# roitberg-group/lammps-ani

Hardware: AMD Instinct MI355X
Metric: MD ns/day for ANI-2x water box (0.5 fs steps; whole timestep loop: integrate + re-neighbour + ghost exchange + pair_style ani hot path) (higher is better)
Workload: dtype f32

## Files before the change

lammps-ani_amd/csrc/ani_handle.h:

```cpp
#pragma once
#include "../../include/ani_hip.h"
#include "../../include/ani_comm.h"

#include <hip/hip_runtime.h>
#ifndef ANI_NO_ROCTX
#include <rocprofiler-sdk-roctx/roctx.h>
#else
static inline void roctxRangePushA(const char*) {}
static inline void roctxRangePop() {}
static inline void roctxMarkA(const char*) {}
#endif

#include <algorithm>
#include <atomic>
#include <chrono>
#include <cmath>
#include <cstdio>
#include <cstdlib>
#include <cstring>
#include <string>
#include <vector>

#include "ani_kernels.h"
#include "ani_model.h"
// ... 43 lines not shown
  std::vector<double*> W64, b64, WT64;
  double *W0c64 = nullptr, *WT0c64 = nullptr, *w_out64 = nullptr, *b_out64 = nullptr;
  struct Planes {
    std::vector<unsigned short*> W, WT;
    unsigned short *W0c = nullptr, *WT0c = nullptr;
  } sp[2];
  std::vector<float> wscale;
  struct Fused {
    unsigned char* stream = nullptr;
    float* consts = nullptr;
    long long ppm = 0;
    int cpm = 0;
  } fu[4];
  int fused_shape = -1;
};
inline MlpArith planes_arith(int i) { return i == 0 ? MLP_BF16X3 : MLP_F16X2; }

struct Options {
  int prune = 1;
  int mlp_pipeline = 0;
  int aev_fused = 1;
  int aev_sym_radial = 1;
  int aev_tickets_min = 40000;
  int aev_stream_tables = 1;
  int mlp_fused_sched = 1;
  int mlp_fused_halves = 1;
  int mlp_fused = 1;
  int mlp_fused_gen = 1;
  int mlp_fused_rows = 0;
  int mlp_chain = 1;
  int profiling = 0;
  int dev_overwrite = 0;
  int mlp_arith = MLP_BF16X3;
  int rdf_lanes = 16, rdf_lds = 1;
  int nbr_onepass = 1, nbr_sorted_rows = 1, nbr_half_cells = 0;
  int reuse_upload = 0;
  int out_force_accumulate = 0;
};

struct FusedState {
  int mask[4] = {-2, -2, -2, -2};
  DevBuf<int> counter;
  DevBuf<int> sched;
  int sched_key[4] = {-1, -1, -1, -1};
  int sched_nitems = 0;
  DevBuf<float> gaev_parts;
// ... 117 lines not shown
  int split_phase = 0;
  hipStream_t side = nullptr;
  hipEvent_t ev_mlp = nullptr, ev_side = nullptr;
  struct { const double* d_x; int eflag_atom, vflag; double *d_f, *d_ev, *d_eatom; } split{};
  int nlocal = 0, ntotal = 0, nrows = 0;
  long long npairs = 0;
  int count[kMaxSpecies] = {0}, row_start[kMaxSpecies] = {0};

  ani_comm* comm = nullptr;
  int sticky_flags = 0;
  int max_numneigh = 0;
  DevBuf<int> species, ilist, numneigh, jlist, jraw, nbr_off, row_of_centre, centre_of_row, bucket_info, err_flag;
  DevBuf<int> row_of_atom;
  DevBuf<unsigned> sym_acc;
  int jraw_stride = 0;
  int jlist_row_stride = 0;
  const int64_t* stage_owner = nullptr;
  const double* stage_shift = nullptr;
  int stage_nghost = -1;
  bool origin_from_box = false;
  GhostFold fold;
  int fold_nghost = -1;
  DevBuf<int> fold_head, fold_next, fold_bad;
  bool warned_asymmetric = false;
  bool list_is_ours = false;
  bool list_symmetric = true;
  DevBuf<int> row_ctr;
  DevBuf<float4> xyzs, cl_xyz;
  DevBuf<int4> row_info, cl_hdr;
  DevBuf<int> cl_j;
  int cl_stride = 0;
  DevBuf<double> x64, f64, ev, eatom, virial_acc;
  DevBuf<double> origin;
  bool need_origin = true;
  DevBuf<double> rep_tables, erep;
  DevBuf<float> aev, gaev, act, e_rows, fbuf;
  DevBuf<double> aev64, gaev64, act64, e_rows64, fbuf64;
  std::vector<std::vector<double*>> Hbuf64;
  std::vector<std::vector<float*>> Hbuf, Gbuf;
  bool arena_valid = false;
};

#define HIP_TRY(h, expr)                                                                              \
  do {                                                                                                \
    hipError_t _e = (expr);                                                                           \
    if (_e != hipSuccess) {                                                                           \
// ... 83 lines not shown
```

lammps-ani_amd/csrc/ani_hip.cpp:

```cpp
#include "ani_handle.h"

namespace ani {
static thread_local hipError_t g_launch_error = hipSuccess;
void note_launch_error(hipError_t e) { if (e != hipSuccess && g_launch_error == hipSuccess) g_launch_error = e; }
hipError_t take_launch_error() { const hipError_t e = g_launch_error; g_launch_error = hipSuccess; return e; }
}

namespace ani_host __attribute__((visibility("hidden"))) {
thread_local std::string g_create_error;
constexpr int kCopyOutBlocks = 32;

int run_step64(ani_handle* h, const double* d_x, int eflag_atom, int vflag, double* d_f, int f_accumulate, double* d_ev,
               double* d_eatom, hipStream_t st) {
  const HostModel& m = h->model;
  const int L = m.L, M = m.M;
  HIP_TRY(h, h->fbuf64.reserve((size_t)std::max(h->ntotal, 1) * 3));
  HIP_TRY(h, h->virial_acc.reserve(9 * kVirialSlots));
  HIP_TRY(h, h->err_flag.reserve(1, true));
  HIP_TRY(h, hipMemsetAsync(h->fbuf64.p, 0, sizeof(double) * 3 * (size_t)h->ntotal, st));
  HIP_TRY(h, hipMemsetAsync(h->virial_acc.p, 0, sizeof(double) * 9, st));
  HIP_TRY(h, hipMemsetAsync(h->e_rows64.p, 0, sizeof(double) * (size_t)M * std::max(h->nrows, 1), st));
  if (h->armed.av_acc) HIP_TRY(h, hipMemsetAsync(h->armed.av_acc, 0, sizeof(double) * 9 * (size_t)h->ntotal, st));
  Aev64Params p{};
  const AevParams& r = h->ap_run;
// ... 208 lines not shown
  StreamTab tab_view;
  const bool rep_done = launch_aev_backward(h->ap_run, a, h->max_numneigh, st, rt.on ? &rt : nullptr, avir, step_stream_tab(h, tab_view)) && rt.on;
  if (m.has_rep && !rep_done) {
    RepArgs ra{};
    ra.row_info = h->row_info.p; ra.nrows = h->nrows; ra.jlist = h->jlist.p; ra.species = h->species.p;
    ra.pos = c.d_x; ra.fbuf = h->fbuf.p; ra.virial = c.vflag ? h->virial_acc.p : nullptr; ra.erep = h->erep.p;
    ra.tables = h->rep_tables.p; ra.S = m.S; ra.nslots = kVirialSlots; ra.vslots = kVirialSlots; ra.cutoff = m.rep_cut;
    launch_repulsion(ra, false, st, avir);
  }
  return ANI_OK;
}

void step_finish(ani_handle* h, const StepCtx& c, int atom0, int atom1, bool energy, hipStream_t st) {
  const HostModel& m = h->model;
  FinishArgs fa{};
  fa.e_rows = h->e_rows.p; fa.M = m.M; fa.nrows = h->nrows; fa.nrows_ld = h->nrows;
  fa.centre_of_row = h->centre_of_row.p; fa.ilist = h->ilist.p; fa.species = h->species.p;
  for (int s = 0; s < m.S; s++) fa.sae[s] = m.sae[s];
  fa.fbuf = h->fbuf.p; fa.atom0 = atom0; fa.atom1 = atom1; fa.energy = energy ? 1 : 0;
  fa.virial_acc = c.vflag ? h->virial_acc.p : nullptr;
  fa.f_out = c.d_f; fa.f_accumulate = c.f_accumulate; fa.ev_out = c.d_ev;
  fa.eatom_out = c.eflag_atom ? c.d_eatom : nullptr;
  fa.err_flag = h->err_flag.p;
  if (h->fold_nghost >= 0 && c.fold) {
    fa.fold_head = h->fold_head.p; fa.fold_next = h->fold_next.p; fa.fold_nlocal = h->nlocal;
    fa.atom1 = std::min(fa.atom1, h->nlocal);
  }
  launch_finish(fa, st);
  if (energy && m.has_rep) launch_repulsion_energy(h->erep.p, kVirialSlots, c.d_ev, st);
}

int run_step(ani_handle* h, const double* d_x, int eflag_atom, int vflag, double* d_f, int f_accumulate, double* d_ev,
             double* d_eatom, hipStream_t st, bool fold = false) {
  if (!h->use_single) return run_step64(h, d_x, eflag_atom, vflag, d_f, f_accumulate, d_ev, d_eatom, st);
  StepCtx c;
  c.fold = fold;
  c.d_x = d_x; c.eflag_atom = eflag_atom; c.vflag = vflag; c.f_accumulate = f_accumulate; c.d_f = d_f; c.d_ev = d_ev; c.d_eatom = d_eatom;
  TraceRange tr_step("ani: step");
  int rc = step_prologue(h, c, true, st);
  if (rc) return rc;
  step_pack(h, c, 0, h->ntotal, true, st);
  if (h->armed.av_acc) HIP_TRY(h, hipMemsetAsync(h->armed.av_acc, 0, sizeof(float) * 9 * (size_t)h->ntotal, st));
  const AevArgs a = step_aev_args(h, c, 0);
  rc = step_compact_forward(h, a, st);
  if (rc) return rc;
  {
    TraceRange tr("ani: MLP forward + backward");
    rc = compute_mlp(h, st);
// ... 170 lines not shown
  for (auto& n : h->nets) {
    for (float* p : n.W) if (p) (void)hipFree(p);
    for (float* p : n.b) if (p) (void)hipFree(p);
    for (float* p : n.WT) if (p) (void)hipFree(p);
    if (n.W0c) (void)hipFree(n.W0c);
    if (n.WT0c) (void)hipFree(n.WT0c);
    if (n.w_out) (void)hipFree(n.w_out);
    if (n.b_out) (void)hipFree(n.b_out);
    for (auto& sp : n.sp) {
      for (unsigned short* p : sp.W) if (p) (void)hipFree(p);
      for (unsigned short* p : sp.WT) if (p) (void)hipFree(p);
      if (sp.W0c) (void)hipFree(sp.W0c);
      if (sp.WT0c) (void)hipFree(sp.WT0c);
    }
    for (double* p : n.W64) if (p) (void)hipFree(p);
    for (double* p : n.b64) if (p) (void)hipFree(p);
    for (double* p : n.WT64) if (p) (void)hipFree(p);
    if (n.W0c64) (void)hipFree(n.W0c64);
    if (n.WT0c64) (void)hipFree(n.WT0c64);
    if (n.w_out64) (void)hipFree(n.w_out64);
    if (n.b_out64) (void)hipFree(n.b_out64);
  }
  h->species.release(); h->ilist.release(); h->numneigh.release(); h->jlist.release(); h->jraw.release(); h->nbr_off.release();
  h->fold_head.release(); h->fold_next.release(); h->fold_bad.release(); h->nb.ovf.release(); h->nb.xq.release(); h->row_of_centre.release(); h->centre_of_row.release(); h->bucket_info.release(); h->err_flag.release(); h->row_ctr.release(); h->row_of_atom.release();
  h->xyzs.release(); h->cl_xyz.release(); h->cl_hdr.release(); h->cl_j.release(); h->row_info.release(); h->row_flag.release(); h->row_list.release(); h->row_count.release(); h->x64.release(); h->f64.release(); h->ev.release(); h->eatom.release(); h->origin.release();
  h->rep_tables.release(); h->erep.release();
  h->nb.cell_id.release(); h->nb.cell_count.release(); h->nb.cell_start.release(); h->nb.cursor.release(); h->nb.order.release(); h->nb.xs.release();
  h->armed.avir.release(); h->armed.avir64.release(); h->armed.avout.release();
  h->armed.gaev_parts64.release(); h->armed.dv_fbuf.release(); h->armed.dv_fbuf64.release(); h->armed.dv_tmp.release(); h->armed.dv_stage.release();
  h->armed.dv_part.release(); h->armed.dv_ticket.release();
  h->mol.bond_cut2.release(); h->mol.ints.release(); h->mol.words.release(); h->mol.owner.release(); h->mol.summary.release(); h->mol.out.release();
  h->rdf.ints.release(); h->rdf.words.release();
  h->virial_acc.release(); h->aev.release(); h->gaev.release(); h->act.release(); h->aev64.release(); h->gaev64.release(); h->act64.release(); h->e_rows64.release(); h->fbuf64.release(); h->e_rows.release(); h->fbuf.release();
  for (int fi = 0; fi < 4; fi++) free_fused(h, fi);
  h->fused.counter.release(); h->fused.gaev_parts.release(); h->fused.sched.release();
  h->stab.desc_b.release(); h->stab.desc_f.release(); h->stab.words_b.release(); h->stab.words_f.release();
  free_chain_plan(h->chain_plan);
  for (auto& e : h->timing.evt_pool) if (e) (void)hipEventDestroy(e);
  if (h->stream) (void)hipStreamDestroy(h->stream);
  delete h;
}

const char* ani_last_error(const ani_handle* h) { return h ? h->err.c_str() : g_create_error.c_str(); }
int ani_num_models(const ani_handle* h) { return h ? h->model.M_file : 0; }
int ani_use_num_models(const ani_handle* h) { return h ? h->model.M : 0; }
int ani_num_species(const ani_handle* h) { return h ? h->model.S : 0; }
int ani_aev_length(const ani_handle* h) { return h ? h->model.aev_len : 0; }
// ... 263 lines not shown
```

lammps-ani_amd/csrc/ani_hip_list.cpp:

```cpp
#include "ani_handle.h"

namespace ani_host __attribute__((visibility("hidden"))) {
constexpr int kRebuildRowsOverflow = -1000;
int rebuild(ani_handle* h, hipStream_t st) {
  const HostModel& m = h->model;
  roctxMarkA("neighbor list rebuilt");
  TraceRange tr("ani: list epoch set-up (offsets, species buckets, segment sort)");
  h->need_origin = !h->origin_from_box;
  h->fold_nghost = -1;
  h->classes_valid = false;
  h->split_phase = 0;
  const int nlocal = h->nlocal;
  const int nrows_cap = round_up(nlocal, kRowTile) + m.S * kRowTile;
  HIP_TRY(h, h->nbr_off.reserve((size_t)nlocal + 1));
  HIP_TRY(h, h->row_of_centre.reserve(prepare_scratch_ints(nlocal)));
  HIP_TRY(h, h->centre_of_row.reserve(nrows_cap));
  HIP_TRY(h, h->row_info.reserve(nrows_cap));
  HIP_TRY(h, h->bucket_info.reserve(kBucketInfoInts));
  HIP_TRY(h, h->err_flag.reserve(1, true));
  if (!h->host.pinned_ints) HIP_TRY(h, hipHostMalloc((void**)&h->host.pinned_ints, sizeof(int) * 32, hipHostMallocDefault));
  h->host.pinned_ints[0] = h->host.pinned_ints[1] = h->host.pinned_ints[2] = 0;
  HIP_TRY(h, hipMemcpyAsync(&h->host.pinned_ints[0], h->err_flag.p, sizeof(int), hipMemcpyDeviceToHost, st));
  HIP_TRY(h, hipMemsetAsync(h->err_flag.p, 0, sizeof(int), st));
  HIP_TRY(h, h->row_of_atom.reserve((size_t)std::max(h->ntotal, 1)));
  PrepOut o{h->nbr_off.p, h->row_of_centre.p, h->centre_of_row.p, h->row_info.p, h->bucket_info.p, h->row_of_atom.p};
  launch_prepare(h->species.p, h->ilist.p, h->numneigh.p, nlocal, h->ntotal, m.S, nrows_cap, o, st, h->jlist_row_stride);
  if (h->jlist_row_stride) HIP_TRY(h, hipMemcpyAsync(&h->host.pinned_ints[1], h->nb.ovf.p, sizeof(int), hipMemcpyDeviceToHost, st));
  const bool fold_staged = h->stage_nghost >= 0 && h->stage_owner && h->use_single && h->stage_nghost == h->ntotal - nlocal;
  if (fold_staged) {
    HIP_TRY(h, h->fold_head.reserve((size_t)std::max(nlocal, 1)));
    HIP_TRY(h, h->fold_next.reserve((size_t)std::max(h->stage_nghost, 1)));
    HIP_TRY(h, h->fold_bad.reserve(1));
    launch_ghost_chain(reinterpret_cast<const long long*>(h->stage_owner), h->stage_nghost, nlocal, h->fold_head.p, h->fold_next.p, h->fold_bad.p, st);
    HIP_TRY(h, hipMemcpyAsync(&h->host.pinned_ints[2], h->fold_bad.p, sizeof(int), hipMemcpyDeviceToHost, st));
  }
  int info[kBucketInfoInts];
  HIP_TRY(h, hipMemcpyAsync(info, h->bucket_info.p, sizeof(info), hipMemcpyDeviceToHost, st));
  HIP_TRY(h, hipStreamSynchronize(st));
  h->sticky_flags |= h->host.pinned_ints[0];
  HIP_TRY(h, take_launch_error());
  if (h->jlist_row_stride && h->host.pinned_ints[1]) return kRebuildRowsOverflow;
  if (h->jlist_row_stride) h->npairs = info[2 * kMaxSpecies + 4];
  if (fold_staged) {
    if (h->host.pinned_ints[2]) { h->stage_nghost = -1; h->err = "ani_stage_ghost_fold: an owner index lies outside [0, nlocal)"; return ANI_ERR_ARG; }
    h->fold.owner = reinterpret_cast<const long long*>(h->stage_owner); h->fold.shift = h->stage_shift; h->fold.nlocal = nlocal;
    h->fold_nghost = h->stage_nghost;
  }
  h->stage_nghost = -1;
  if (info[2 * kMaxSpecies + 1]) { h->err = "an atom has a species outside the model's species list (or ilist holds an index outside [0, ntotal))"; return ANI_ERR_ARG; }
  for (int s = 0; s < m.S; s++) { h->count[s] = info[s]; h->row_start[s] = info[kMaxSpecies + s]; }
  h->nrows = info[2 * kMaxSpecies];
  h->max_numneigh = info[2 * kMaxSpecies + 2];
  {
    const int rcs = specialize(h, info[2 * kMaxSpecies + 3]);
    if (rcs) return rcs;
    const int rct = build_stream_tables(h, st);
// ... 218 lines not shown
  h->host.species32.resize(ntotal);
  for (int i = 0; i < ntotal; i++) h->host.species32[i] = (int)species[i];
  HIP_TRY(h, h->species.reserve(ntotal));
  HIP_TRY(h, h->x64.reserve((size_t)ntotal * 3));
  HIP_TRY(h, hipMemcpyAsync(h->species.p, h->host.species32.data(), sizeof(int) * (size_t)ntotal, hipMemcpyHostToDevice, st));
  HIP_TRY(h, hipMemcpyAsync(h->x64.p, coordinates, sizeof(double) * 3 * (size_t)ntotal, hipMemcpyHostToDevice, st));
  const int rcb = build_list(h, ntotal, nlocal, h->species.p, h->x64.p, cutneigh, lo, hi, out_npairs, st);
  h->host.x64_from = (rcb == ANI_OK && h->opt.reuse_upload) ? coordinates : nullptr;
  return rcb;
}

int ani_set_ghost_fold(ani_handle* h, const int64_t* d_owner, const double* d_shift, int nghost, void* stream) {
  if (!h) return ANI_ERR_ARG;
  if (!d_owner || nghost < 0) { h->fold_nghost = -1; return ANI_OK; }
  if (!h->use_single) { h->err = "ani_set_ghost_fold: the fp64 kernels do not fold ghosts (use the exchange kernels)"; return ANI_ERR_ARG; }
  if (!h->have_list || nghost != h->ntotal - h->nlocal) { h->err = "ani_set_ghost_fold: no list installed, or nghost differs from the list's"; return ANI_ERR_ARG; }
  if (!d_shift && nghost > 0) { h->err = "ani_set_ghost_fold: null shift"; return ANI_ERR_ARG; }
  HIP_TRY(h, hipSetDevice(h->device));
  hipStream_t st = (hipStream_t)stream;
  HIP_TRY(h, h->fold_head.reserve((size_t)std::max(h->nlocal, 1)));
  HIP_TRY(h, h->fold_next.reserve((size_t)std::max(nghost, 1)));
  HIP_TRY(h, h->fold_bad.reserve(1));
  static_assert(sizeof(long long) == sizeof(int64_t), "owner indices are 64-bit");
  launch_ghost_chain(reinterpret_cast<const long long*>(d_owner), nghost, h->nlocal, h->fold_head.p, h->fold_next.p, h->fold_bad.p, st);
  int bad = 0;
  HIP_TRY(h, hipMemcpyAsync(&bad, h->fold_bad.p, sizeof(int), hipMemcpyDeviceToHost, st));
  HIP_TRY(h, hipStreamSynchronize(st));
  HIP_TRY(h, take_launch_error());
  if (bad) { h->fold_nghost = -1; h->err = "ani_set_ghost_fold: an owner index lies outside [0, nlocal)"; return ANI_ERR_ARG; }
  h->fold.owner = reinterpret_cast<const long long*>(d_owner); h->fold.shift = d_shift; h->fold.nlocal = h->nlocal;
  h->fold_nghost = nghost;
  return ANI_OK;
}

int ani_stage_ghost_fold(ani_handle* h, const int64_t* d_owner, const double* d_shift, int nghost) {
  if (!h) return ANI_ERR_ARG;
  h->stage_owner = nullptr; h->stage_shift = nullptr; h->stage_nghost = -1;
  if (!d_owner || nghost < 0) return ANI_OK;
  if (!h->use_single) { h->err = "ani_stage_ghost_fold: the fp64 kernels do not fold ghosts (use the exchange kernels)"; return ANI_ERR_ARG; }
  if (!d_shift && nghost > 0) { h->err = "ani_stage_ghost_fold: null shift"; return ANI_ERR_ARG; }
  h->stage_owner = d_owner; h->stage_shift = d_shift; h->stage_nghost = nghost;
  return ANI_OK;
}
}
```

lammps-ani_amd/csrc/ani_hip_options.cpp:

```cpp
#include "ani_handle.h"

extern "C" {
void ani_trace_push(const char* name) { if (name) roctxRangePushA(name); }
void ani_trace_pop(void) { roctxRangePop(); }
void ani_trace_mark(const char* name) { if (name) roctxMarkA(name); }

const char* ani_last_mlp_kernel(const ani_handle* h) { return h ? h->last_mlp_kernel : ""; }

int ani_debug_get(ani_handle* h, ani_debug_view* out) {
  if (!h || !out) return ANI_ERR_ARG;
  memset(out, 0, sizeof(*out));
  out->nlocal = h->nlocal; out->ntotal = h->ntotal; out->nrows = h->nrows; out->npairs = h->npairs;
  out->d_aev = h->aev.p; out->d_gaev = h->gaev.p; out->d_row_of_centre = h->row_of_centre.p;
  out->aev_stride = h->ap_run.aev_stride; out->aev_active_length = h->ap_run.aev_len;
  if (h->err_flag.p) {
    int flag = 0;
    if (hipSetDevice(h->device) == hipSuccess && hipDeviceSynchronize() == hipSuccess &&
        hipMemcpy(&flag, h->err_flag.p, sizeof(int), hipMemcpyDeviceToHost) == hipSuccess)
      h->sticky_flags |= flag;
  }
  out->error_flags = h->sticky_flags;
  for (int s = 0; s < kMaxSpecies && s < 16; s++) out->species_count[s] = h->count[s];
  return ANI_OK;
}
// ... 39 lines not shown
  for (int c = 0; c < h->ap_run.aev_len && c < (int)h->colmap.size(); c++) out[c] = h->colmap[c];
  return ANI_OK;
}

enum OptKind { kFlag, kRange, kSet };
enum OptInvalidates { kNothing, kSchedule, kList, kUpload };
struct OptRow { const char* name; int Options::*field; OptKind kind; int v[3]; const char* refusal; OptInvalidates invalidates; };
constexpr int kAny = 0x7fffffff;
static const OptRow kOptionRows[] = {
    {"prune_absent_species", &Options::prune, kFlag, {}, nullptr, kList},
    {"rdf_lanes", &Options::rdf_lanes, kSet, {16, 64, 64}, "ani_set_option: rdf_lanes is 16 or 64", kNothing},
    {"rdf_lds", &Options::rdf_lds, kFlag, {}, nullptr, kNothing},
    {"mlp_chain", &Options::mlp_chain, kRange, {-kAny - 1, kAny}, nullptr, kNothing},
    {"nbr_onepass", &Options::nbr_onepass, kFlag, {}, nullptr, kNothing},
    {"out_force_accumulate", &Options::out_force_accumulate, kFlag, {}, nullptr, kNothing},
    {"nbr_sorted_rows", &Options::nbr_sorted_rows, kFlag, {}, nullptr, kNothing},
    {"nbr_half_cells", &Options::nbr_half_cells, kFlag, {}, nullptr, kNothing},
    {"reuse_build_list_upload", &Options::reuse_upload, kFlag, {}, nullptr, kUpload},
    {"mlp_fused", &Options::mlp_fused, kRange, {0, 3}, "mlp_fused must be 0, 1, 2 or 3", kNothing},
    {"aev_symmetric_radial", &Options::aev_sym_radial, kFlag, {}, nullptr, kNothing},
    {"aev_tickets_min", &Options::aev_tickets_min, kRange, {0, kAny}, "aev_tickets_min must be >= 0", kNothing},
    {"aev_fused", &Options::aev_fused, kFlag, {}, nullptr, kNothing},
    {"aev_stream_tables", &Options::aev_stream_tables, kFlag, {}, nullptr, kNothing},
    {"mlp_fused_gen", &Options::mlp_fused_gen, kRange, {0, 1}, "mlp_fused_gen must be 0 or 1", kSchedule},
    {"mlp_fused_rows", &Options::mlp_fused_rows, kSet, {0, 64, 128}, "mlp_fused_rows must be 0, 64 or 128", kSchedule},
    {"mlp_fused_halves", &Options::mlp_fused_halves, kRange, {0, 2}, "mlp_fused_halves must be 0, 1 or 2", kSchedule},
    {"mlp_fused_schedule", &Options::mlp_fused_sched, kFlag, {}, nullptr, kSchedule},
    {"mlp_pipeline", &Options::mlp_pipeline, kRange, {0, 2}, "mlp_pipeline must be 0, 1 or 2", kNothing},
    {"mlp_arith", &Options::mlp_arith, kRange, {0, 2}, "mlp_arith must be 0 (fp32-input MFMA), 1 (bf16 x 3, exact) or 2 (fp16 x 2)", kNothing},
    {"mlp_split_bf16", &Options::mlp_arith, kFlag, {}, nullptr, kNothing},
    {"device_overwrite_forces", &Options::dev_overwrite, kFlag, {}, nullptr, kNothing},
    {"profiling", &Options::profiling, kFlag, {}, nullptr, kNothing},
    {"full_radial_capacity", nullptr, kFlag, {}, nullptr, kNothing},
};
static_assert(MLP_FP32 == 0 && MLP_BF16X3 == 1, "mlp_split_bf16 is a flag onto mlp_arith");

int ani_set_option(ani_handle* h, const char* name, int value) {
  if (!h || !name) return ANI_ERR_ARG;
  for (const OptRow& r : kOptionRows) {
    if (strcmp(name, r.name) != 0) continue;
    const bool ok = r.kind == kFlag || (r.kind == kRange ? value >= r.v[0] && value <= r.v[1] : value == r.v[0] || value == r.v[1] || value == r.v[2]);
    if (!ok) { h->err = r.refusal; return ANI_ERR_ARG; }
    const int stored = r.kind == kFlag ? value != 0 : value;
    if (r.field) h->opt.*r.field = stored;
    else h->ap.full_cap = h->ap_run.full_cap = stored;
    if (r.invalidates == kSchedule) h->fused.sched_key[0] = -1;
// ... 92 lines not shown
```

lammps-ani_amd/csrc/ani_kernels.h:

```cpp
#pragma once
#include <hip/hip_runtime.h>

#include <cstdint>
#include <vector>

#include "ani_fused_host.h"
#include "ani_model.h"

namespace ani {

constexpr int kRowTile = 128;
constexpr int kMaxRad = 256;
constexpr int kMaxAng = 96;
constexpr int kBucketInfoInts = 2 * kMaxSpecies + 5;
constexpr int kVirialSlots = 1024;

enum Epilogue { EPI_PLAIN = 0, EPI_CELU = 1, EPI_LAST = 2, EPI_BWD = 3 };

void note_launch_error(hipError_t e);
hipError_t take_launch_error();
int device_num_cus();
hipError_t raise_dynamic_lds(const void* kernel, int bytes);

struct GemmArgs {
// ... 70 lines not shown
void launch_build_stream(const float* src, int ld, int rows_valid, int k_valid, int NT, int KS, int chunk, int P, float scale,
                         unsigned short* dst, hipStream_t st);
hipError_t launch_mlp_fused(const FusedArgs& G, MlpArith arith, hipStream_t st);
hipError_t launch_mlp_fused16(const FusedArgs& G, MlpArith arith, int waves, hipStream_t st);
int fused16_b1_chunks(int nt0);
int fused16_b1_chunk_tiles(int nt0, int ci);
void launch_build_stream16(const float* src, int ld, int rows_valid, int k_valid, int NT, int KS, int order, int nt_off, int identity,
                           int P, float scale, unsigned short* dst, hipStream_t st);
void launch_sum_parts(const float* parts, long long part_stride, int M, float* dst, long long n, hipStream_t st);
int aev_read_stamps(unsigned long long* out32, int reset);
int fused_read_stamps(unsigned long long* out16, int reset);

void launch_split_planes(const float* src, int batch, long long s_src, int N, int K, int ld, MlpArith arith, float scale,
                         unsigned short* dst, hipStream_t st);
inline size_t split_elems(int N, int K, MlpArith arith) { return (size_t)N * ((K + 15) / 16) * 16 * mlp_planes(arith); }

struct SpeciesMap { int m[kMaxSpecies]; };
void launch_origin(const double* d_x, int ntotal, double* d_origin, hipStream_t st);
struct GhostFold {
  const long long* owner = nullptr;
  const double* shift = nullptr;
  int nlocal = 0;
};
void launch_ghost_chain(const long long* d_owner, int nghost, int nlocal, int* d_head, int* d_next, int* d_bad, hipStream_t st);
void launch_pack(const double* d_x, const int* d_species, int i0, int i1, const SpeciesMap& cmap, float4* xyzs, float* fbuf,
                 double* virial_acc, double* ev_zero, const double* d_origin, hipStream_t st, const GhostFold* gf = nullptr);
void launch_row_classes(const int4* row_info, const int* jlist, int nrows, int nlocal, int* flag, int* list, int* count, hipStream_t st);

void launch_step_tail(const double* d_ev, const int* d_flag, double* host_out, double stamp, hipStream_t st);
void launch_copy_out(const double* d_f, double* host, long long n, int nchunks, unsigned long long* d_ctr, unsigned* host_flags,
                     unsigned epoch, int nblocks, hipStream_t st);

struct PrepOut {
  int* nbr_off;
  int* row_of_centre;
  int* centre_of_row;
  int4* row_info;
  int* bucket_info;
  int* row_of_atom;
};
size_t prepare_scratch_ints(int nlocal);
void launch_prepare(const int* d_species, const int* d_ilist, const int* d_numneigh, int nlocal, int ntotal, int S, int nrows_cap,
                    const PrepOut& o, hipStream_t st, int row_stride = 0);
void launch_list_symmetry(const int* d_ilist, const int* d_nbr_off, const int* d_numneigh, const int* d_jraw, const int* d_row_of_atom,
                          int nlocal, int ntotal, unsigned* d_acc, int* d_out, hipStream_t st);

constexpr int kTicketGroups = 64;
constexpr int kTicketMaxGroups = 256;
static_assert(kTicketGroups <= kTicketMaxGroups, "kTicketGroups");
constexpr int kTicketStride = 64;
struct AevArgs {
  const float4* xyzs;
  const int* ilist;
  const int* numneigh;
  const int* nbr_off;
  const int* jlist;
  const int* centre_of_row;
  const int4* row_info;
  int nrows;
  float* aev;
  const float* gaev;
  float* fbuf;
  double* virial;
  int* err_flag;
  int4* cl_hdr;
  float4* cl_xyz;
// ... 74 lines not shown
};
void launch_repulsion(const RepArgs& a, bool fp64, hipStream_t st, void* avir = nullptr);
void launch_repulsion_energy(const double* erep, int nslots, double* d_ev, hipStream_t st);

struct FinishArgs {
  const float* e_rows;
  int M, nrows, nrows_ld;
  const int* centre_of_row;
  const int* ilist;
  const int* species;
  double sae[kMaxSpecies];
  const float* fbuf;
  int atom0, atom1;
  int energy;
  const double* virial_acc;
  double* f_out;
  int f_accumulate;
  double* ev_out;
  double* eatom_out;
  const int* err_flag;
  const int* fold_head = nullptr;
  const int* fold_next = nullptr;
  int fold_nlocal = 0;
};
void launch_finish(const FinishArgs& a, hipStream_t st);
void launch_atom_virial(const void* acc, bool fp64, int natoms, int ncomp, double* out, int accumulate, const int* fold_head,
                        const int* fold_next, int fold_nlocal, hipStream_t st);

void launch_dev_parts(float* parts, long long part_stride, int M, float* dst, long long n, int sum, hipStream_t st);
void launch_dev_parts64(double* parts, long long part_stride, int M, const double* dst, long long n, hipStream_t st);
void launch_dev_member(void* acc, bool fp64, int nrows_out, int nlocal, int m, int M, double* dforce, double* dsq, const int* fold_head,
                       const int* fold_next, int fold_nlocal, hipStream_t st);
constexpr int kDevEnergyParts = 32;
struct DevCloseArgs {
  const void* e_rows;
  int M, nrows, nrows_ld, nlocal;
  const int* centre_of_row;
  const int* ilist;
  const int* species;
  double sae[kMaxSpecies];
  const double* erep;
  int nslots;
  const double* dsq;
  double* member_energy;
  double* atom_energy_dev;
  double* atom_force_dev;
// ... 94 lines not shown
```

lammps-ani_amd/csrc/ani_kernels_misc.hip:

```cpp
#include <mutex>
#include <set>
#include <utility>

#include "ani_kernels.h"
#include "ani_scan.h"

namespace ani {

int device_num_cus() {
  static const int ncu = [] {
    int dev = 0, v = 256;
    if (hipGetDevice(&dev) == hipSuccess) note_launch_error(hipDeviceGetAttribute(&v, hipDeviceAttributeMultiprocessorCount, dev));
    return v > 0 ? v : 256;
  }();
  return ncu;
}

hipError_t raise_dynamic_lds(const void* kernel, int bytes) {
  static std::set<std::pair<int, const void*>> raised;
  static std::mutex mtx;
  int dev = 0;
  hipError_t e = hipGetDevice(&dev);
  if (e != hipSuccess) return e;
  std::lock_guard<std::mutex> lock(mtx);
// ... 57 lines not shown
  }
  out[i] = make_float4((float)(px - origin[0]), (float)(py - origin[1]), (float)(pz - origin[2]), __int_as_float(cs));
  reinterpret_cast<float4*>(fbuf)[i] = make_float4(0.f, 0.f, 0.f, 0.f);
}

void launch_pack(const double* d_x, const int* d_species, int i0, int i1, const SpeciesMap& cmap, float4* xyzs, float* fbuf,
                 double* virial_acc, double* ev_zero, const double* d_origin, hipStream_t st, const GhostFold* gf) {
  int nthr = i1 - i0;
  if (virial_acc && nthr < 9 * kVirialSlots) nthr = 9 * kVirialSlots;
  if (ev_zero && nthr < 10) nthr = 10;
  if (nthr <= 0) return;
  hipLaunchKernelGGL(pack_kernel, dim3((nthr + 255) / 256), dim3(256), 0, st, d_x, d_species, i0, i1, cmap,
                     xyzs, fbuf, virial_acc, ev_zero, d_origin, gf ? *gf : GhostFold{});
}

__global__ __launch_bounds__(256) void ghost_chain_kernel(const long long* __restrict__ owner, int nghost, int nlocal, int* __restrict__ head,
                                                          int* __restrict__ next, int* __restrict__ bad) {
  const int g = blockIdx.x * blockDim.x + threadIdx.x;
  if (g >= nghost) return;
  const long long o = owner[g];
  if (o < 0 || o >= nlocal) { *bad = 1; next[g] = -1; return; }
  next[g] = atomicExch(head + o, g);
}
void launch_ghost_chain(const long long* d_owner, int nghost, int nlocal, int* d_head, int* d_next, int* d_bad, hipStream_t st) {
  note_launch_error(hipMemsetAsync(d_head, 0xff, sizeof(int) * (size_t)(nlocal > 0 ? nlocal : 1), st));
  note_launch_error(hipMemsetAsync(d_bad, 0, sizeof(int), st));
  if (nghost > 0) hipLaunchKernelGGL(ghost_chain_kernel, dim3((nghost + 255) / 256), dim3(256), 0, st, d_owner, nghost, nlocal, d_head, d_next, d_bad);
}

__global__ void step_tail_kernel(const double* __restrict__ ev, const int* __restrict__ flag, volatile double* __restrict__ host_out,
                                 double stamp) {
  const int t = threadIdx.x;
  if (t < 10) host_out[t] = ev[t];
  if (t == 10) host_out[10] = (double)*flag;
  __threadfence_system();
  __syncthreads();
  if (t == 0) { host_out[11] = stamp; __threadfence_system(); }
}
void launch_step_tail(const double* d_ev, const int* d_flag, double* host_out, double stamp, hipStream_t st) {
  hipLaunchKernelGGL(step_tail_kernel, dim3(1), dim3(64), 0, st, d_ev, d_flag, host_out, stamp);
}

__global__ __launch_bounds__(256) void copy_out_kernel(const double* __restrict__ f, double* __restrict__ host, long long n, int nchunks,
                                                       unsigned long long* __restrict__ ctr, volatile unsigned* __restrict__ host_flags,
                                                       unsigned epoch) {
  const double2* __restrict__ f2 = reinterpret_cast<const double2*>(f);
  double2* __restrict__ h2 = reinterpret_cast<double2*>(host);
  for (int c = 0; c < nchunks; c++) {
    const long long a = (n * c / nchunks) & ~1LL, b = c + 1 == nchunks ? n : ((n * (c + 1) / nchunks) & ~1LL);
    const long long len2 = (b - a) >> 1;
// ... 99 lines not shown
      o.bucket_info[2 * kMaxSpecies] = r;
    }
  }
  __syncthreads();
  const int ii = blockIdx.x * blockDim.x + threadIdx.x;
  if (ii >= nlocal) {
    if (nlocal == 0 && ii == 0) o.nbr_off[0] = 0;
    return;
  }
  const int len = numneigh[ii];
  const int off = row_stride > 0 ? ii * row_stride : before[0] + o.nbr_off[ii];
  o.nbr_off[ii] = off;
  if (ii == nlocal - 1) o.nbr_off[nlocal] = row_stride > 0 ? nlocal * row_stride : off + len;
  const int i = ilist[ii];
  const int sp = (i >= 0 && i < ntotal) ? species[i] : -1;
  if (sp < 0 || sp >= S) { o.row_of_centre[ii] = -1; return; }
  const int row = row_start[sp] + before[1 + sp] + rank_in_species[ii];
  o.row_of_centre[ii] = row;
  if (row < nrows_cap) {
    o.centre_of_row[row] = ii;
    o.row_info[row] = make_int4(i, off, len, ii);
    if (o.row_of_atom) o.row_of_atom[i] = row;
  }
}

size_t prepare_scratch_ints(int nlocal) {
  return (size_t)2 * nlocal + ((size_t)nlocal / kPrepChunk + 1) * (kMaxSpecies + 1) + 2;
}

void launch_prepare(const int* d_species, const int* d_ilist, const int* d_numneigh, int nlocal, int ntotal, int S, int nrows_cap,
                    const PrepOut& o, hipStream_t st, int row_stride) {
  int* rank = o.row_of_centre + nlocal;
  int* chunk_tot = o.row_of_centre + 2 * (size_t)nlocal;
  const int nchunks = nlocal / kPrepChunk + 1;
  note_launch_error(hipMemsetAsync(o.centre_of_row, 0xff, sizeof(int) * (size_t)nrows_cap, st));
  note_launch_error(hipMemsetAsync(o.row_info, 0xff, sizeof(int4) * (size_t)nrows_cap, st));
  note_launch_error(hipMemsetAsync(o.bucket_info, 0, sizeof(int) * kBucketInfoInts, st));
  if (o.row_of_atom) note_launch_error(hipMemsetAsync(o.row_of_atom, 0xff, sizeof(int) * (size_t)(ntotal > 0 ? ntotal : 1), st));
  hipLaunchKernelGGL(prepare_count_kernel, dim3(nchunks), dim3(1024), 0, st, d_species, d_ilist, d_numneigh, nlocal, ntotal, S, o,
                     rank, chunk_tot);
  hipLaunchKernelGGL(prepare_rows_kernel, dim3(nlocal > 0 ? (nlocal + 255) / 256 : 1), dim3(256), 0, st, d_species, d_ilist,
                     d_numneigh, nlocal, ntotal, S, nrows_cap, o, rank, chunk_tot, row_stride);
}

__device__ __forceinline__ unsigned pair_hash(unsigned a, unsigned b) {
  const unsigned lo = a < b ? a : b, hi = a < b ? b : a;
// ... 19 lines not shown
  }
  for (int o = 32; o > 0; o >>= 1) own += __shfl_xor(own, o);
  if (lane == 0 && own) atomicAdd(acc + i, own);
}
__global__ __launch_bounds__(256) void list_symmetry_verdict_kernel(const unsigned* __restrict__ acc, int ntotal, int* __restrict__ out) {
  const int i = blockIdx.x * blockDim.x + threadIdx.x;
  if (i < ntotal && acc[i] != 0u) atomicOr(out, 1);
}
void launch_list_symmetry(const int* d_ilist, const int* d_nbr_off, const int* d_numneigh, const int* d_jraw, const int* d_row_of_atom,
                          int nlocal, int ntotal, unsigned* d_acc, int* d_out, hipStream_t st) {
  note_launch_error(hipMemsetAsync(d_acc, 0, sizeof(unsigned) * (size_t)(ntotal > 0 ? ntotal : 1), st));
  note_launch_error(hipMemsetAsync(d_out, 0, sizeof(int), st));
  if (nlocal <= 0) return;
  hipLaunchKernelGGL(list_symmetry_kernel, dim3((nlocal + 3) / 4), dim3(256), 0, st, d_ilist, d_nbr_off, d_numneigh, d_jraw, d_row_of_atom,
                     nlocal, ntotal, d_acc);
  hipLaunchKernelGGL(list_symmetry_verdict_kernel, dim3((ntotal + 255) / 256), dim3(256), 0, st, d_acc, ntotal, d_out);
}

constexpr int kFinishBlocks = 128;

__global__ __launch_bounds__(256) void finish_kernel(FinishArgs a) {
  __shared__ double red[256];
  const int b = a.energy ? blockIdx.x : blockIdx.x + kFinishBlocks + 1;
  if (b < kFinishBlocks) {
    double acc = 0.0;
    for (int row = b * blockDim.x + threadIdx.x; row < a.nrows; row += kFinishBlocks * blockDim.x) {
      const int ii = a.centre_of_row[row];
      if (ii < 0) continue;
      float e = 0.f;
      for (int m = 0; m < a.M; m++) e += a.e_rows[(long long)m * a.nrows_ld + row];
      const double ea = (double)e + a.sae[a.species[a.ilist[ii]]];
      if (a.eatom_out) a.eatom_out[ii] = ea * 627.5094738898777;
      acc += ea;
    }
    red[threadIdx.x] = acc;
    __syncthreads();
    for (int s = 128; s > 0; s >>= 1) {
      if ((int)threadIdx.x < s) red[threadIdx.x] += red[threadIdx.x + s];
      __syncthreads();
    }
    if (threadIdx.x == 0) {
      const bool bad = b == 0 && a.err_flag && *a.err_flag;
      atomicAdd(&a.ev_out[0], bad ? __longlong_as_double(0x7ff8000000000000LL) : red[0] * 627.5094738898777);
    }
    return;
  }
// ... 2 lines not shown
    __shared__ double vsum[9];
    for (int c = 0; c < 9; c++) {
      double t = 0.0;
      for (int sl = threadIdx.x; sl < kVirialSlots; sl += blockDim.x) t += a.virial_acc[9 * sl + c];
      red[threadIdx.x] = t;
      __syncthreads();
      for (int s2 = 128; s2 > 0; s2 >>= 1) {
        if ((int)threadIdx.x < s2) red[threadIdx.x] += red[threadIdx.x + s2];
        __syncthreads();
      }
      if (threadIdx.x == 0) vsum[c] = red[0];
      __syncthreads();
    }
    if (threadIdx.x < 9) {
      const int k = threadIdx.x / 3, l = threadIdx.x % 3;
      a.ev_out[1 + threadIdx.x] = 0.5 * (vsum[3 * k + l] + vsum[3 * l + k]) * 627.5094738898777;
    }
    return;
  }
  const int i = 3 * a.atom0 + (b - kFinishBlocks - 1) * blockDim.x + threadIdx.x;
  if (i >= 3 * a.atom1) return;
  const int at = i / 3, c = i - 3 * at;
  float acc = a.fbuf[4 * at + c];
  if (a.fold_head) {
    for (int g = a.fold_head[at]; g >= 0; g = a.fold_next[g]) acc += a.fbuf[4 * (a.fold_nlocal + g) + c];
  }
  const double v = (double)acc * 627.5094738898777;
  a.f_out[i] = a.f_accumulate ? a.f_out[i] + v : v;
}

void launch_finish(const FinishArgs& a, hipStream_t st) {
  const int n3 = a.f_out ? (a.atom1 - a.atom0) * 3 : 0;
  const int blocks = (a.energy ? kFinishBlocks + 1 : 0) + (n3 + 255) / 256;
  if (blocks <= 0) return;
  hipLaunchKernelGGL(finish_kernel, dim3(blocks), dim3(256), 0, st, a);
}

template <typename T>
__global__ __launch_bounds__(256) void atom_virial_kernel(const T* __restrict__ acc, int natoms, int ncomp, double* __restrict__ out,
                                                          int accumulate, const int* __restrict__ fold_head,
                                                          const int* __restrict__ fold_next, int fold_nlocal) {
  const int i = blockIdx.x * blockDim.x + threadIdx.x;
  if (i >= natoms) return;
  double s[9];
#pragma unroll
  for (int k = 0; k < 9; k++) s[k] = (double)acc[9 * (long long)i + k];
  if (fold_head) {
// ... 307 lines not shown
```

Measured before the change: 64.43.

## Precompute per-row SAE and flatten ghost-fold chains into spans for finish kernel

At re-neighbour time, a new kernel precomputes each row's self-atomic energy and their total. A second new kernel turns the linked-list ghost chains into contiguous span/index arrays. The finish kernel then sums energies with 4-way unrolled independent loads instead of a dependent species/ilist lookup per row, and folds ghost forces through the flat index arrays instead of pointer-chasing the chain. The aim is lower latency in the per-step finish kernel, paid for with extra kernels and memsets at list rebuild and a change in floating-point summation order.

```diff
diff --git a/lammps-ani_amd/csrc/ani_handle.h b/lammps-ani_amd/csrc/ani_handle.h
--- a/lammps-ani_amd/csrc/ani_handle.h
+++ b/lammps-ani_amd/csrc/ani_handle.h
@@ -89,6 +89,7 @@
   int aev_fused = 1;
   int aev_sym_radial = 1;
   int aev_tickets_min = 40000;
+  int finish_rows = 1;
   int aev_stream_tables = 1;
   int mlp_fused_sched = 1;
   int mlp_fused_halves = 1;
@@ -252,6 +253,9 @@
   GhostFold fold;
   int fold_nghost = -1;
   DevBuf<int> fold_head, fold_next, fold_bad;
+  DevBuf<int2> fold_span;
+  DevBuf<int> fold_idx;
+  DevBuf<double> sae_rows;
   bool warned_asymmetric = false;
   bool list_is_ours = false;
   bool list_symmetric = true;
diff --git a/lammps-ani_amd/csrc/ani_hip.cpp b/lammps-ani_amd/csrc/ani_hip.cpp
--- a/lammps-ani_amd/csrc/ani_hip.cpp
+++ b/lammps-ani_amd/csrc/ani_hip.cpp
@@ -254,8 +254,10 @@
   fa.f_out = c.d_f; fa.f_accumulate = c.f_accumulate; fa.ev_out = c.d_ev;
   fa.eatom_out = c.eflag_atom ? c.d_eatom : nullptr;
   fa.err_flag = h->err_flag.p;
+  if (h->opt.finish_rows && h->sae_rows.p) { fa.sae_sum = h->sae_rows.p; fa.sae_row = h->sae_rows.p + 1; }
   if (h->fold_nghost >= 0 && c.fold) {
     fa.fold_head = h->fold_head.p; fa.fold_next = h->fold_next.p; fa.fold_nlocal = h->nlocal;
+    if (h->opt.finish_rows) { fa.fold_span = h->fold_span.p; fa.fold_idx = h->fold_idx.p; }
     fa.atom1 = std::min(fa.atom1, h->nlocal);
   }
   launch_finish(fa, st);
@@ -472,7 +474,7 @@
     if (n.b_out64) (void)hipFree(n.b_out64);
   }
   h->species.release(); h->ilist.release(); h->numneigh.release(); h->jlist.release(); h->jraw.release(); h->nbr_off.release();
-  h->fold_head.release(); h->fold_next.release(); h->fold_bad.release(); h->nb.ovf.release(); h->nb.xq.release(); h->row_of_centre.release(); h->centre_of_row.release(); h->bucket_info.release(); h->err_flag.release(); h->row_ctr.release(); h->row_of_atom.release();
+  h->fold_head.release(); h->fold_next.release(); h->fold_bad.release(); h->fold_span.release(); h->fold_idx.release(); h->sae_rows.release(); h->nb.ovf.release(); h->nb.xq.release(); h->row_of_centre.release(); h->centre_of_row.release(); h->bucket_info.release(); h->err_flag.release(); h->row_ctr.release(); h->row_of_atom.release();
   h->xyzs.release(); h->cl_xyz.release(); h->cl_hdr.release(); h->cl_j.release(); h->row_info.release(); h->row_flag.release(); h->row_list.release(); h->row_count.release(); h->x64.release(); h->f64.release(); h->ev.release(); h->eatom.release(); h->origin.release();
   h->rep_tables.release(); h->erep.release();
   h->nb.cell_id.release(); h->nb.cell_count.release(); h->nb.cell_start.release(); h->nb.cursor.release(); h->nb.order.release(); h->nb.xs.release();
diff --git a/lammps-ani_amd/csrc/ani_hip_list.cpp b/lammps-ani_amd/csrc/ani_hip_list.cpp
--- a/lammps-ani_amd/csrc/ani_hip_list.cpp
+++ b/lammps-ani_amd/csrc/ani_hip_list.cpp
@@ -25,13 +25,20 @@
   HIP_TRY(h, h->row_of_atom.reserve((size_t)std::max(h->ntotal, 1)));
   PrepOut o{h->nbr_off.p, h->row_of_centre.p, h->centre_of_row.p, h->row_info.p, h->bucket_info.p, h->row_of_atom.p};
   launch_prepare(h->species.p, h->ilist.p, h->numneigh.p, nlocal, h->ntotal, m.S, nrows_cap, o, st, h->jlist_row_stride);
+  if (h->use_single) {
+    HIP_TRY(h, h->sae_rows.reserve((size_t)nrows_cap + 1));
+    launch_row_sae(h->centre_of_row.p, h->ilist.p, h->species.p, m.sae.data(), m.S, nrows_cap, h->sae_rows.p + 1, h->sae_rows.p, st);
+  }
   if (h->jlist_row_stride) HIP_TRY(h, hipMemcpyAsync(&h->host.pinned_ints[1], h->nb.ovf.p, sizeof(int), hipMemcpyDeviceToHost, st));
   const bool fold_staged = h->stage_nghost >= 0 && h->stage_owner && h->use_single && h->stage_nghost == h->ntotal - nlocal;
   if (fold_staged) {
     HIP_TRY(h, h->fold_head.reserve((size_t)std::max(nlocal, 1)));
     HIP_TRY(h, h->fold_next.reserve((size_t)std::max(h->stage_nghost, 1)));
     HIP_TRY(h, h->fold_bad.reserve(1));
-    launch_ghost_chain(reinterpret_cast<const long long*>(h->stage_owner), h->stage_nghost, nlocal, h->fold_head.p, h->fold_next.p, h->fold_bad.p, st);
+    HIP_TRY(h, h->fold_span.reserve((size_t)std::max(nlocal, 0) + 1));
+    HIP_TRY(h, h->fold_idx.reserve((size_t)std::max(h->stage_nghost, 1)));
+    launch_ghost_chain(reinterpret_cast<const long long*>(h->stage_owner), h->stage_nghost, nlocal, h->fold_head.p, h->fold_next.p, h->fold_bad.p, st,
+                       h->fold_span.p, h->fold_idx.p);
     HIP_TRY(h, hipMemcpyAsync(&h->host.pinned_ints[2], h->fold_bad.p, sizeof(int), hipMemcpyDeviceToHost, st));
   }
   int info[kBucketInfoInts];
@@ -296,7 +303,10 @@
   HIP_TRY(h, h->fold_next.reserve((size_t)std::max(nghost, 1)));
   HIP_TRY(h, h->fold_bad.reserve(1));
   static_assert(sizeof(long long) == sizeof(int64_t), "owner indices are 64-bit");
-  launch_ghost_chain(reinterpret_cast<const long long*>(d_owner), nghost, h->nlocal, h->fold_head.p, h->fold_next.p, h->fold_bad.p, st);
+  HIP_TRY(h, h->fold_span.reserve((size_t)std::max(h->nlocal, 0) + 1));
+  HIP_TRY(h, h->fold_idx.reserve((size_t)std::max(nghost, 1)));
+  launch_ghost_chain(reinterpret_cast<const long long*>(d_owner), nghost, h->nlocal, h->fold_head.p, h->fold_next.p, h->fold_bad.p, st,
+                     h->fold_span.p, h->fold_idx.p);
   int bad = 0;
   HIP_TRY(h, hipMemcpyAsync(&bad, h->fold_bad.p, sizeof(int), hipMemcpyDeviceToHost, st));
   HIP_TRY(h, hipStreamSynchronize(st));
diff --git a/lammps-ani_amd/csrc/ani_hip_options.cpp b/lammps-ani_amd/csrc/ani_hip_options.cpp
--- a/lammps-ani_amd/csrc/ani_hip_options.cpp
+++ b/lammps-ani_amd/csrc/ani_hip_options.cpp
@@ -85,6 +85,7 @@
     {"aev_tickets_min", &Options::aev_tickets_min, kRange, {0, kAny}, "aev_tickets_min must be >= 0", kNothing},
     {"aev_fused", &Options::aev_fused, kFlag, {}, nullptr, kNothing},
     {"aev_stream_tables", &Options::aev_stream_tables, kFlag, {}, nullptr, kNothing},
+    {"finish_rows", &Options::finish_rows, kFlag, {}, nullptr, kNothing},
     {"mlp_fused_gen", &Options::mlp_fused_gen, kRange, {0, 1}, "mlp_fused_gen must be 0 or 1", kSchedule},
     {"mlp_fused_rows", &Options::mlp_fused_rows, kSet, {0, 64, 128}, "mlp_fused_rows must be 0, 64 or 128", kSchedule},
     {"mlp_fused_halves", &Options::mlp_fused_halves, kRange, {0, 2}, "mlp_fused_halves must be 0, 1 or 2", kSchedule},
diff --git a/lammps-ani_amd/csrc/ani_kernels.h b/lammps-ani_amd/csrc/ani_kernels.h
--- a/lammps-ani_amd/csrc/ani_kernels.h
+++ b/lammps-ani_amd/csrc/ani_kernels.h
@@ -116,7 +116,8 @@
   const double* shift = nullptr;
   int nlocal = 0;
 };
-void launch_ghost_chain(const long long* d_owner, int nghost, int nlocal, int* d_head, int* d_next, int* d_bad, hipStream_t st);
+void launch_ghost_chain(const long long* d_owner, int nghost, int nlocal, int* d_head, int* d_next, int* d_bad, hipStream_t st,
+                        int2* d_span = nullptr, int* d_idx = nullptr);
 void launch_pack(const double* d_x, const int* d_species, int i0, int i1, const SpeciesMap& cmap, float4* xyzs, float* fbuf,
                  double* virial_acc, double* ev_zero, const double* d_origin, hipStream_t st, const GhostFold* gf = nullptr);
 void launch_row_classes(const int4* row_info, const int* jlist, int nrows, int nlocal, int* flag, int* list, int* count, hipStream_t st);
@@ -136,6 +137,8 @@
 size_t prepare_scratch_ints(int nlocal);
 void launch_prepare(const int* d_species, const int* d_ilist, const int* d_numneigh, int nlocal, int ntotal, int S, int nrows_cap,
                     const PrepOut& o, hipStream_t st, int row_stride = 0);
+void launch_row_sae(const int* d_centre_of_row, const int* d_ilist, const int* d_species, const double* sae, int S, int nrows_cap,
+                    double* d_sae_row, double* d_sae_sum, hipStream_t st);
 void launch_list_symmetry(const int* d_ilist, const int* d_nbr_off, const int* d_numneigh, const int* d_jraw, const int* d_row_of_atom,
                           int nlocal, int ntotal, unsigned* d_acc, int* d_out, hipStream_t st);
 
@@ -256,6 +259,10 @@
   const int* fold_head = nullptr;
   const int* fold_next = nullptr;
   int fold_nlocal = 0;
+  const double* sae_row = nullptr;
+  const double* sae_sum = nullptr;
+  const int2* fold_span = nullptr;
+  const int* fold_idx = nullptr;
 };
 void launch_finish(const FinishArgs& a, hipStream_t st);
 void launch_atom_virial(const void* acc, bool fp64, int natoms, int ncomp, double* out, int accumulate, const int* fold_head,
diff --git a/lammps-ani_amd/csrc/ani_kernels_misc.hip b/lammps-ani_amd/csrc/ani_kernels_misc.hip
--- a/lammps-ani_amd/csrc/ani_kernels_misc.hip
+++ b/lammps-ani_amd/csrc/ani_kernels_misc.hip
@@ -103,10 +103,26 @@
   if (o < 0 || o >= nlocal) { *bad = 1; next[g] = -1; return; }
   next[g] = atomicExch(head + o, g);
 }
-void launch_ghost_chain(const long long* d_owner, int nghost, int nlocal, int* d_head, int* d_next, int* d_bad, hipStream_t st) {
+__global__ __launch_bounds__(256) void ghost_spans_kernel(const int* __restrict__ head, const int* __restrict__ next, int nlocal,
+                                                          int nghost, int2* __restrict__ span, int* __restrict__ idx,
+                                                          int* __restrict__ cursor) {
+  const int i = blockIdx.x * blockDim.x + threadIdx.x;
+  if (i >= nlocal) return;
+  int n = 0;
+  for (int g = head[i]; g >= 0; g = next[g]) n++;
+  int k = n ? atomicAdd(cursor, n) : 0;
+  span[i] = make_int2(k, n);
+  for (int g = head[i]; g >= 0 && k < nghost; g = next[g]) idx[k++] = g;
+}
+void launch_ghost_chain(const long long* d_owner, int nghost, int nlocal, int* d_head, int* d_next, int* d_bad, hipStream_t st,
+                        int2* d_span, int* d_idx) {
   note_launch_error(hipMemsetAsync(d_head, 0xff, sizeof(int) * (size_t)(nlocal > 0 ? nlocal : 1), st));
   note_launch_error(hipMemsetAsync(d_bad, 0, sizeof(int), st));
   if (nghost > 0) hipLaunchKernelGGL(ghost_chain_kernel, dim3((nghost + 255) / 256), dim3(256), 0, st, d_owner, nghost, nlocal, d_head, d_next, d_bad);
+  if (!d_span || !d_idx || nlocal <= 0) return;
+  int* cursor = reinterpret_cast<int*>(d_span + nlocal);
+  note_launch_error(hipMemsetAsync(cursor, 0, sizeof(int2), st));
+  hipLaunchKernelGGL(ghost_spans_kernel, dim3((nlocal + 255) / 256), dim3(256), 0, st, d_head, d_next, nlocal, nghost, d_span, d_idx, cursor);
 }
 
 __global__ void step_tail_kernel(const double* __restrict__ ev, const int* __restrict__ flag, volatile double* __restrict__ host_out,
@@ -252,6 +268,36 @@
     o.row_info[row] = make_int4(i, off, len, ii);
     if (o.row_of_atom) o.row_of_atom[i] = row;
   }
+}
+
+struct SaeTab { double v[kMaxSpecies]; };
+__global__ __launch_bounds__(256) void row_sae_kernel(const int* __restrict__ centre_of_row, const int* __restrict__ ilist,
+                                                      const int* __restrict__ species, SaeTab sae, int nrows_cap,
+                                                      double* __restrict__ sae_row, double* __restrict__ sae_sum) {
+  __shared__ double red[256];
+  const int row = blockIdx.x * blockDim.x + threadIdx.x;
+  double v = 0.0;
+  if (row < nrows_cap) {
+    const int ii = centre_of_row[row];
+    if (ii >= 0) v = sae.v[species[ilist[ii]]];
+    sae_row[row] = v;
+  }
+  red[threadIdx.x] = v;
+  __syncthreads();
+  for (int s = 128; s > 0; s >>= 1) {
+    if ((int)threadIdx.x < s) red[threadIdx.x] += red[threadIdx.x + s];
+    __syncthreads();
+  }
+  if (threadIdx.x == 0 && red[0] != 0.0) atomicAdd(sae_sum, red[0]);
+}
+void launch_row_sae(const int* d_centre_of_row, const int* d_ilist, const int* d_species, const double* sae, int S, int nrows_cap,
+                    double* d_sae_row, double* d_sae_sum, hipStream_t st) {
+  note_launch_error(hipMemsetAsync(d_sae_sum, 0, sizeof(double), st));
+  if (nrows_cap <= 0) return;
+  SaeTab t{};
+  for (int s = 0; s < S && s < kMaxSpecies; s++) t.v[s] = sae[s];
+  hipLaunchKernelGGL(row_sae_kernel, dim3((nrows_cap + 255) / 256), dim3(256), 0, st, d_centre_of_row, d_ilist, d_species, t, nrows_cap,
+                     d_sae_row, d_sae_sum);
 }
 
 size_t prepare_scratch_ints(int nlocal) {
@@ -317,6 +363,42 @@
 __global__ __launch_bounds__(256) void finish_kernel(FinishArgs a) {
   __shared__ double red[256];
   const int b = a.energy ? blockIdx.x : blockIdx.x + kFinishBlocks + 1;
+  if (b < kFinishBlocks && a.sae_row) {
+    double acc = 0.0;
+    const int stride = kFinishBlocks * blockDim.x;
+    for (int row0 = b * blockDim.x + threadIdx.x; row0 < a.nrows; row0 += 4 * stride) {
+      int ii[4];
+      float e[4];
+      double sr[4];
+#pragma unroll
+      for (int k = 0; k < 4; k++) {
+        const long long row = (long long)row0 + (long long)k * stride;
+        const bool in = row < a.nrows;
+        ii[k] = in ? a.centre_of_row[row] : -1;
+        e[k] = 0.f;
+        for (int m = 0; m < a.M; m++) e[k] += in ? a.e_rows[(long long)m * a.nrows_ld + row] : 0.f;
+        sr[k] = (in && a.eatom_out) ? a.sae_row[row] : 0.0;
+      }
+#pragma unroll
+      for (int k = 0; k < 4; k++) {
+        if (ii[k] < 0) continue;
+        if (a.eatom_out) a.eatom_out[ii[k]] = ((double)e[k] + sr[k]) * 627.5094738898777;
+        acc += (double)e[k];
+      }
+    }
+    red[threadIdx.x] = acc;
+    __syncthreads();
+    for (int s = 128; s > 0; s >>= 1) {
+      if ((int)threadIdx.x < s) red[threadIdx.x] += red[threadIdx.x + s];
+      __syncthreads();
+    }
+    if (threadIdx.x == 0) {
+      const bool bad = b == 0 && a.err_flag && *a.err_flag;
+      const double share = b == 0 ? red[0] + *a.sae_sum : red[0];
+      atomicAdd(&a.ev_out[0], bad ? __longlong_as_double(0x7ff8000000000000LL) : share * 627.5094738898777);
+    }
+    return;
+  }
   if (b < kFinishBlocks) {
     double acc = 0.0;
     for (int row = b * blockDim.x + threadIdx.x; row < a.nrows; row += kFinishBlocks * blockDim.x) {
@@ -365,7 +447,18 @@
   if (i >= 3 * a.atom1) return;
   const int at = i / 3, c = i - 3 * at;
   float acc = a.fbuf[4 * at + c];
-  if (a.fold_head) {
+  if (a.fold_span) {
+    const int2 sp = a.fold_span[at];
+    const int o1 = sp.x + sp.y;
+    for (int o = sp.x; o < o1; o += 4) {
+      float t[4];
+#pragma unroll
+      for (int k = 0; k < 4; k++) t[k] = o + k < o1 ? a.fbuf[4 * ((long long)a.fold_nlocal + a.fold_idx[o + k]) + c] : 0.f;
+#pragma unroll
+      for (int k = 0; k < 4; k++)
+        if (o + k < o1) acc += t[k];
+    }
+  } else if (a.fold_head) {
     for (int g = a.fold_head[at]; g >= 0; g = a.fold_next[g]) acc += a.fbuf[4 * (a.fold_nlocal + g) + c];
   }
   const double v = (double)acc * 627.5094738898777;
```

New measurement: 64.53 (median of 3 runs). About the same (+0.2%).
